# cvlab-yonsei/HVPR

Hardware: AMD Instinct MI355X
Metric: KITTI frames/sec/GPU (fwd, ~20k pts); VFE+scatter achieved HBM GB/s vs peak (higher is better)
Workload: dtype f32; 1 GPU; hvpr_car.yaml batch=1 forward-only, a1..a8 (on-GPU voxelize, pillar VFE, memory read-out + scatter, BEV backbone, head + decode, score top-k + rotated-BEV NMS); frames sharded over ranks, replicas only; global_batch=1, weights=deterministic synthetic (seed 0), BN stats randomised, cls bias -4.595

## Files before the change

### hvpr_amd/csrc/conv_wino.hip

```cpp
#include <type_traits>

#include "common.h"
#include "wino_walk.h"

namespace {

typedef float f32x16 __attribute__((ext_vector_type(16)));
constexpr int KC = 8;
constexpr int BN = 64;
constexpr int TW = 16, PW = TW + 2;
constexpr int ROWP = 20;
constexpr int W_V4 = 16 * 2 * BN;

__device__ __forceinline__ void lds_dma16(const void *sbase_uniform, unsigned voff_bytes, unsigned lds_dst_uniform) {
    unsigned keep;
    asm volatile("s_mov_b32 %0, m0\n\ts_mov_b32 m0, %3\n\ts_nop 0\n\tglobal_load_lds_dwordx4 %1, %2\n\ts_mov_b32 m0, %0"
                 : "=&s"(keep)
                 : "v"(voff_bytes), "s"(sbase_uniform), "s"(lds_dst_uniform)
                 : "memory");
}

__device__ __forceinline__ unsigned lds_addr_of(const void *p) {
    return (unsigned)(size_t)(const __attribute__((address_space(3))) void *)p;
}

struct WinoArgs {
    const float *in;
    const float *wpk;
    const float *bias;
    float *out;
    const float *gate;
    const float *resid;
    int N, H, W, Cin;
    int cout, cout_pad;
    int out_cstride, out_coff, resid_cstride;
    int relu;
    WinoWalk walk;
    int n_ct;
    float *stats;
};

__device__ __forceinline__ float4 f4_fma(float s, float4 a, float4 b) {
    return make_float4(fmaf(s, a.x, b.x), fmaf(s, a.y, b.y), fmaf(s, a.z, b.z), fmaf(s, a.w, b.w));
}
__device__ __forceinline__ float4 f4_add(float4 a, float4 b) { return make_float4(a.x + b.x, a.y + b.y, a.z + b.z, a.w + b.w); }
__device__ __forceinline__ float4 f4_sub(float4 a, float4 b) { return make_float4(a.x - b.x, a.y - b.y, a.z - b.z, a.w - b.w); }

template <int NG, bool STATS, int NB>
__global__ void __launch_bounds__(256 * NG) __attribute__((amdgpu_waves_per_eu(2, NB == 2 ? 2 : 3))) k_wino(WinoArgs a) {
    constexpr int NT = 256 * NG;
    constexpr int TH = 8 * NG, PH = TH + 2;
    constexpr int PPAD = (PH * ROWP + 63) / 64 * 64;
    constexpr int PATCH_V4 = 2 * PPAD;
    constexpr int BNT = 32 * NB, W_V4T = 16 * 2 * BNT;
    constexpr int NLD_P = (PATCH_V4 + NT - 1) / NT, NLD_W = W_V4T / NT;
    constexpr int PATCH_PAD = NLD_P * NT;
    constexpr bool PAIR = NG == 1 && NB == 2 && !STATS;
    constexpr int PH_S = PAIR ? 12 : PH, PW_S = PAIR ? 20 : PW;
    constexpr int BIAS_SLOT = PH_S * ROWP;
    static_assert(W_V4T % NT == 0 && (NB == 2 || NG == 1), "whole DMA pieces");
    extern __shared__ __attribute__((aligned(16))) float4 smem[];
    float4 *const s_w = smem;
    float4 *const s_patch = smem + 2 * W_V4T;

    const int tid = threadIdx.x, lane = tid & 63, wid = tid >> 6;
    const unsigned wave_s = __builtin_amdgcn_readfirstlane((unsigned)(threadIdx.x >> 6));
    const int grp = wid >> 2, wa = wid & 3;
    const int half = lane >> 5, l31 = lane & 31;
    const int by = l31 >> 3, bx = l31 & 7;

    int p_py[NLD_P], p_px[NLD_P], p_part[NLD_P];
    bool p_live[NLD_P], p_one[NLD_P];
#pragma unroll
    for (int i = 0; i < NLD_P; ++i) {
        const int v = tid + i * NT;
        const int plane = v / PPAD, slot = v % PPAD;
        const int y = slot / ROWP, rem = slot % ROWP;
        const int x = 2 * (rem % 10) + rem / 10;
        p_py[i] = y; p_px[i] = x; p_part[i] = plane * 4;
        p_live[i] = plane < 2 && y < PH_S && x < PW_S;
        p_one[i] = plane < 2 && y < PH && x < PW;
    }
    const int r0 = wa == 0 ? 0 : (wa == 2 ? 2 : 1), r1 = wa == 2 ? 1 : (wa == 3 ? 3 : 2);
    const float sgn = wa == 1 ? 1.f : -1.f;
    const int pbase = half * PPAD + (2 * (4 * grp + by)) * ROWP + bx;
    const int u_off = (wa * 4 * 2 + half) * BNT + l31;
    const unsigned lds_w0 = lds_addr_of(s_w) + wave_s * 1024u;
    const unsigned lds_patch0 = lds_addr_of(s_patch) + wave_s * 1024u;

    const int n_pt = a.walk.per_image * a.N;
    const int total_walk = ((n_pt + 7) / 8) * 8 * a.n_ct;
    const int n_chunks = a.Cin / KC;
    for (int it = blockIdx.x; it < total_walk; it += gridDim.x) {
    int ct;
    int pt = wino_walk_step(it, a.n_ct, ct);
    if (pt >= n_pt) continue;
    int tx, ty, n, mode = WINO_SINGLE;
    if constexpr (PAIR) {
        const WinoItem w = wino_walk_item(a.walk, pt);
        tx = w.tx; ty = w.ty; n = w.n; mode = w.mode;
    } else {
        tx = pt % a.walk.tiles_x; pt /= a.walk.tiles_x;
        ty = pt % a.walk.tiles_y;
        n = pt / a.walk.tiles_y;
    }
    const bool pr = PAIR && mode == WINO_PAIR_RIGHT, pb = PAIR && mode == WINO_PAIR_BOTTOM;
    const bool lane_b = pr ? bx >= 4 : (pb && by >= 2);
    const int p_off0 = pbase + r0 * ROWP + (lane_b ? (pr ? 1 : 2 * ROWP) : 0), p_off1 = p_off0 + (r1 - r0) * ROWP;
    const int oy0 = ty * TH, ox0 = tx * TW;
    const int iy0 = oy0 - 1, ix0 = ox0 - 1;
    const int co0 = ct * BNT;

    unsigned poff[NLD_P];
    bool pok[NLD_P];
#pragma unroll
    for (int i = 0; i < NLD_P; ++i) {
        int iy = iy0 + p_py[i], ix = ix0 + p_px[i];
        bool ok = PAIR ? p_one[i] : p_live[i];
        if (pr) { ok = p_live[i] && p_py[i] < PH; if (p_px[i] >= 10) { iy += TH; ix -= 10; } }
        if (pb) { ok = p_live[i] && p_px[i] < PW; if (p_py[i] >= 6) { iy -= 6; ix += TW; } }
        pok[i] = ok && iy >= 0 && iy < a.H && ix >= 0 && ix < a.W;
        poff[i] = pok[i] ? (unsigned)(((iy * a.W + ix) * a.Cin + p_part[i]) * (int)sizeof(float)) : 0u;
    }
    const char *in_n = (const char *)(a.in + (size_t)n * a.H * a.W * a.Cin);
    const char *w_ct = (const char *)(a.wpk + (size_t)(NB == 2 ? ct : ct >> 1) * n_chunks * (W_V4 * 4));
    const unsigned w_half = NB == 2 ? 0u : (unsigned)(ct & 1) * 32u * 16u;

    auto stage_piece = [&](int chunk, int buf, int i) {
        if (i < NLD_P) {
            const char *pbase_g = in_n + (size_t)chunk * (KC * sizeof(float));
            if (pok[i]) lds_dma16(pbase_g, poff[i], lds_patch0 + (unsigned)(buf * PATCH_PAD + i * NT) * 16u);
        } else {
            const int j = i - NLD_P;
            const char *wbase = w_ct + (size_t)chunk * (W_V4 * 16);
            lds_dma16(wbase, NB == 2 ? (unsigned)((tid + j * NT) * 16) : (unsigned)((((tid + j * NT) >> 5) * 64 + ((tid + j * NT) & 31)) * 16) + w_half,
                      lds_w0 + (unsigned)(buf * W_V4T + j * NT) * 16u);
        }
    };
    auto stage = [&](int chunk, int buf) {
#pragma unroll
        for (int i = 0; i < NLD_P + NLD_W; ++i) stage_piece(chunk, buf, i);
    };
    const bool border = pr || pb || iy0 < 0 || ix0 < 0 || iy0 + PH > a.H || ix0 + PW > a.W;
    if (border) {
#pragma unroll
        for (int b = 0; b < 2; ++b)
#pragma unroll
            for (int i = 0; i < NLD_P; ++i) s_patch[b * PATCH_PAD + tid + i * NT] = make_float4(0.f, 0.f, 0.f, 0.f);
        __syncthreads();
    }
    static_assert(BIAS_SLOT + BNT / 4 <= PPAD, "room for the bias row behind the patch");
    if (tid < BNT / 4) s_patch[BIAS_SLOT + tid] = *(const float4 *)(a.bias + co0 + tid * 4);
    f32x16 acc[4][NB];
#pragma unroll
    for (int b = 0; b < 4; ++b)
#pragma unroll
        for (int nb = 0; nb < NB; ++nb)
#pragma unroll
            for (int r = 0; r < 16; ++r) acc[b][nb][r] = 0.f;

    auto chunk_step = [&](int c, auto buf_tag) {
        constexpr int BUF = decltype(buf_tag)::value;
        asm volatile("s_waitcnt vmcnt(0)" ::: "memory");
        __builtin_amdgcn_s_barrier();
        const float4 *sp = s_patch + BUF * PATCH_PAD;
        const float4 *sw = s_w + BUF * W_V4T;
        float4 d0[4], d1[4], u[4][NB];
#pragma unroll
        for (int jx = 0; jx < 4; ++jx) {
            d0[jx] = sp[p_off0 + (jx & 1) * 10 + (jx >> 1)];
            d1[jx] = sp[p_off1 + (jx & 1) * 10 + (jx >> 1)];
        }
#pragma unroll
        for (int b = 0; b < 2; ++b)
#pragma unroll
            for (int nb = 0; nb < NB; ++nb) u[b][nb] = sw[u_off + b * 2 * BNT + nb * 32];
        __builtin_amdgcn_sched_barrier(0);
        float4 t[4], v[4];
#pragma unroll
        for (int jx = 0; jx < 4; ++jx) t[jx] = f4_fma(sgn, d1[jx], d0[jx]);
        v[0] = f4_sub(t[0], t[2]); v[1] = f4_add(t[1], t[2]); v[2] = f4_sub(t[2], t[1]); v[3] = f4_sub(t[1], t[3]);
#pragma unroll
        for (int b = 0; b < 4; ++b) {
            if (b + 2 < 4) {
#pragma unroll
                for (int nb = 0; nb < NB; ++nb) u[b + 2][nb] = sw[u_off + (b + 2) * 2 * BNT + nb * 32];
            }
            __builtin_amdgcn_sched_barrier(0);
#pragma unroll
            for (int nb = 0; nb < NB; ++nb) {
                acc[b][nb] = __builtin_amdgcn_mfma_f32_32x32x2f32(u[b][nb].x, v[b].x, acc[b][nb], 0, 0, 0);
                acc[b][nb] = __builtin_amdgcn_mfma_f32_32x32x2f32(u[b][nb].y, v[b].y, acc[b][nb], 0, 0, 0);
                acc[b][nb] = __builtin_amdgcn_mfma_f32_32x32x2f32(u[b][nb].z, v[b].z, acc[b][nb], 0, 0, 0);
                acc[b][nb] = __builtin_amdgcn_mfma_f32_32x32x2f32(u[b][nb].w, v[b].w, acc[b][nb], 0, 0, 0);
                constexpr int DEAL = 4 * NB > 5 ? 5 : 4 * NB - 1, NPF = (NLD_P + NLD_W + DEAL - 1) / DEAL;
                static_assert(DEAL * NPF >= NLD_P + NLD_W, "every piece goes out");
                if (c + 1 < n_chunks && b * NB + nb < DEAL) {
                    __builtin_amdgcn_sched_barrier(0);
#pragma unroll
                    for (int i = (b * NB + nb) * NPF; i < (b * NB + nb + 1) * NPF && i < NLD_P + NLD_W; ++i) stage_piece(c + 1, BUF ^ 1, i);
                    __builtin_amdgcn_sched_barrier(0);
                }
            }
            __builtin_amdgcn_sched_barrier(0);
        }
    };
    stage(0, 0);
    for (int c = 0; c + 1 < n_chunks; c += 2) {
        chunk_step(c, std::integral_constant<int, 0>{});
        chunk_step(c + 1, std::integral_constant<int, 1>{});
    }
    if (n_chunks & 1) chunk_step(n_chunks - 1, std::integral_constant<int, 0>{});

    const int p = wa >> 1, q = wa & 1;
    const int oy = oy0 + 2 * (4 * grp + by) + p + (lane_b ? (pr ? TH : -4) : 0), ox = ox0 + 2 * bx + q + (lane_b ? (pr ? -8 : TW) : 0);
    const bool live_px = oy < a.H && ox < a.W;
    const size_t pix = ((size_t)n * a.H + (live_px ? oy : 0)) * a.W + (live_px ? ox : 0);
    const float gate = a.gate && live_px ? a.gate[pix] : 0.f;
    const float *rrow = a.gate ? a.resid + pix * a.resid_cstride : nullptr;
    const float sg = p ? -1.f : 1.f;
    constexpr int NPASS = NG == 1 ? 1 : 2, NBP = NB / NPASS;
    float4 ykeep[2][4];
#pragma unroll
    for (int i = 0; i < 8; ++i) ykeep[i >> 2][i & 3] = make_float4(0.f, 0.f, 0.f, 0.f);
#pragma unroll
    for (int ps = 0; ps < NPASS; ++ps) {
        __syncthreads();
#pragma unroll
        for (int nl = 0; nl < NBP; ++nl) {
            const int nb = ps * NBP + nl;
#pragma unroll
            for (int g = 0; g < 4; ++g) {
                float4 m[4];
#pragma unroll
                for (int b = 0; b < 4; ++b) m[b] = make_float4(acc[b][nb][4 * g], acc[b][nb][4 * g + 1], acc[b][nb][4 * g + 2], acc[b][nb][4 * g + 3]);
                s_w[((((grp * 4 + wa) * 2 + 0) * NBP + nl) * 4 + g) * 64 + lane] = f4_add(f4_add(m[0], m[1]), m[2]);
                s_w[((((grp * 4 + wa) * 2 + 1) * NBP + nl) * 4 + g) * 64 + lane] = f4_sub(f4_sub(m[1], m[2]), m[3]);
            }
        }
        __syncthreads();
        if (live_px) {
#pragma unroll
            for (int nl = 0; nl < NBP; ++nl) {
                const int nb = ps * NBP + nl;
#pragma unroll
                for (int g = 0; g < 4; ++g) {
                    const int col = co0 + nb * 32 + 8 * g + 4 * half;
                    if (col >= a.cout) continue;
                    const float4 x0 = s_w[((((grp * 4 + p) * 2 + q) * NBP + nl) * 4 + g) * 64 + lane];
                    const float4 x1 = s_w[((((grp * 4 + p + 1) * 2 + q) * NBP + nl) * 4 + g) * 64 + lane];
                    const float4 x2 = s_w[((((grp * 4 + p + 2) * 2 + q) * NBP + nl) * 4 + g) * 64 + lane];
                    const float4 bias = s_patch[BIAS_SLOT + (col - co0) / 4];
                    float4 y = f4_add(f4_fma(sg, x2, f4_fma(sg, x1, x0)), bias);
                    if (a.relu) { y.x = fmaxf(y.x, 0.f); y.y = fmaxf(y.y, 0.f); y.z = fmaxf(y.z, 0.f); y.w = fmaxf(y.w, 0.f); }
                    if (a.gate) {
                        const float4 r = *(const float4 *)(rrow + col);
                        y.x = fmaf(gate, y.x, r.x); y.y = fmaf(gate, y.y, r.y); y.z = fmaf(gate, y.z, r.z); y.w = fmaf(gate, y.w, r.w);
                    }
                    *(float4 *)(a.out + pix * a.out_cstride + a.out_coff + col) = y;
                    if (STATS) ykeep[nl][g] = y;
                }
            }
        }
    }
    static_assert(!STATS || (NG == 1 && NB == 2), "the statistics pass is written for the 8 x 16 px x 64 channel tile");
    if (STATS) {
        __syncthreads();
#pragma unroll
        for (int nl = 0; nl < 2; ++nl)
#pragma unroll
            for (int g = 0; g < 4; ++g) s_w[((wid * 2 + nl) * 4 + g) * 64 + lane] = ykeep[nl][g];
        __syncthreads();
        {
            const int c = tid & 63, part = tid >> 6;
            const float *base = (const float *)(s_w + ((part * 2 + (c >> 5)) * 4 + ((c >> 3) & 3)) * 64 + ((c >> 2) & 1) * 32) + (c & 3);
            float sm = 0.f, sq = 0.f;
#pragma unroll 8
            for (int i = 0; i < 32; ++i) {
                const float v = base[((i + c) & 31) * 4];
                sm += v; sq = fmaf(v, v, sq);
            }
            float *s_part = (float *)(s_w + 2048);
            s_part[(part * 2 + 0) * 64 + c] = sm;
            s_part[(part * 2 + 1) * 64 + c] = sq;
        }
        __syncthreads();
        if (tid < 128) {
            const float *s_part = (const float *)(s_w + 2048);
            const int c = tid & 63, k = tid >> 6;
            const float v = (s_part[(0 * 2 + k) * 64 + c] + s_part[(1 * 2 + k) * 64 + c]) + (s_part[(2 * 2 + k) * 64 + c] + s_part[(3 * 2 + k) * 64 + c]);
            const int pt_lin = (n * a.walk.tiles_y + ty) * a.walk.tiles_x + tx;
            if (co0 + c < a.cout) a.stats[((size_t)pt_lin * 2 + k) * a.cout + co0 + c] = v;
        }
    }
    __syncthreads();
    }
}

__global__ void k_wino_pack(const float *__restrict__ w, const float *__restrict__ scale, int cout, int cin, int cout_pad, int adjoint,
                            float *__restrict__ out) {
    const long long id = blockIdx.x * (long long)blockDim.x + threadIdx.x;
    if (id >= (long long)cout_pad * cin) return;
    const int o = (int)(id / cin), i = (int)(id % cin);
    double g[3][3];
#pragma unroll
    for (int u = 0; u < 3; ++u)
#pragma unroll
        for (int v = 0; v < 3; ++v) {
            double x = 0.0;
            if (o < cout) x = adjoint ? (double)w[(((size_t)i * cout + o) * 3 + (2 - u)) * 3 + (2 - v)] : (double)w[(((size_t)o * cin + i) * 3 + u) * 3 + v];
            g[u][v] = (scale && o < cout) ? x * (double)scale[o] : x;
        }
    double gg[4][3];
#pragma unroll
    for (int v = 0; v < 3; ++v) {
        gg[0][v] = g[0][v];
        gg[1][v] = 0.5 * (g[0][v] + g[1][v] + g[2][v]);
        gg[2][v] = 0.5 * (g[0][v] - g[1][v] + g[2][v]);
        gg[3][v] = g[2][v];
    }
    const int ct = o / BN, co_l = o % BN, chunk = i / KC, hf = (i % KC) / 4, e = i % 4;
    float *dst = out + ((size_t)ct * (cin / KC) + chunk) * (W_V4 * 4);
#pragma unroll
    for (int r = 0; r < 4; ++r) {
        const double U[4] = {gg[r][0], 0.5 * (gg[r][0] + gg[r][1] + gg[r][2]), 0.5 * (gg[r][0] - gg[r][1] + gg[r][2]), gg[r][2]};
#pragma unroll
        for (int b = 0; b < 4; ++b) dst[(((size_t)(r * 4 + b) * 2 + hf) * BN + co_l) * 4 + e] = (float)U[b];
    }
}

template <int NG, bool STATS, int NB>
int launch(WinoArgs a, hipStream_t s) {
    constexpr int NT = 256 * NG, TH = 8 * NG, PH = TH + 2;
    constexpr int PPAD = (PH * ROWP + 63) / 64 * 64;
    constexpr int NLD_P = (2 * PPAD + NT - 1) / NT;
    constexpr int lds = (2 * (16 * 2 * 32 * NB) + 2 * NLD_P * NT) * 16;
    a.walk = wino_walk_make(a.H, a.W, TH, NG == 1 && NB == 2 && !STATS);
    a.n_ct = a.cout_pad / (32 * NB);
    static unsigned long long lds_set = 0ull;
    if (hvpr_ensure_dyn_lds((const void *)k_wino<NG, STATS, NB>, lds, &lds_set) != 0) return -1;
    const long long tiles = (long long)a.N * a.walk.per_image * a.n_ct;
    static int resident = 0;
    if (resident == 0) {
        int per_cu = 0, dev = 0, cus = 256;
        hipDeviceProp_t prop;
        if (hipGetDevice(&dev) == hipSuccess && hipGetDeviceProperties(&prop, dev) == hipSuccess) cus = prop.multiProcessorCount;
        if (hipOccupancyMaxActiveBlocksPerMultiprocessor(&per_cu, k_wino<NG, STATS, NB>, NT, lds) != hipSuccess || per_cu < 1) per_cu = 1;
        resident = per_cu * cus;
    }
    long long blocks = tiles < resident ? (tiles + 7) / 8 * 8 : resident;
    if (blocks > resident && resident >= 8) blocks = resident / 8 * 8;
    hipLaunchKernelGGL((k_wino<NG, STATS, NB>), dim3((unsigned)blocks), dim3(NT), lds, s, a);
    return 0;
}

}

extern "C" int hvpr_conv2d_wino_stats_rows(int N, int H, int W) {
    if (N < 1 || H < 1 || W < 1) return 0;
    return N * ((H + 7) / 8) * ((W + TW - 1) / TW);
}

extern "C" int hvpr_conv2d_wino_items(int N, int H, int W, int cout, int px_groups) {
    if (N < 1 || H < 1 || W < 1 || cout < 1 || (px_groups != 1 && px_groups != 2 && px_groups != 4)) return 0;
    const WinoWalk w = wino_walk_make(H, W, px_groups == 2 ? 16 : 8, px_groups == 1);
    const long long items = (long long)N * w.per_image * ((cout + BN - 1) / BN * BN / (px_groups == 4 ? 32 : 64));
    return items < (1ll << 31) ? (int)items : 0;
}

extern "C" size_t hvpr_conv2d_wino_packed_floats(int cin, int cout) {
    if (cin < 1 || cout < 1) return 0;
    return (size_t)((cout + BN - 1) / BN * BN) * (size_t)cin * 16;
}

extern "C" int hvpr_conv2d_wino_pack_f32(const float *weight, const float *scale, int cout, int cin, int adjoint, float *packed,
                                         hvpr_stream_t stream) {
    if (!weight || !packed || cout < 1 || cin < 1) return HVPR_ERR_INVALID_ARG;
    if (cin % KC != 0) return HVPR_ERR_UNSUPPORTED;
    const int cout_pad = (cout + BN - 1) / BN * BN;
    const long long n = (long long)cout_pad * cin;
    hipLaunchKernelGGL(k_wino_pack, dim3(hvpr_cdiv(n, 256)), dim3(256), 0, (hipStream_t)stream, weight, scale, cout, cin, cout_pad,
                       adjoint ? 1 : 0, packed);
    HVPR_CHECK_LAUNCH();
    return HVPR_OK;
}

extern "C" int hvpr_conv2d_wino_nhwc_f32(const float *in, int N, int H, int W, int Cin, const float *w_packed, const float *bias,
                                         int cout, int relu, const float *gate, const float *resid, int resid_cstride, float *out,
                                         int out_cstride, int out_coff, int px_groups, float *bn_partials, hvpr_stream_t stream) {
    if (!in || !w_packed || !bias || !out || N < 1 || H < 1 || W < 1 || Cin < 8 || cout < 1) return HVPR_ERR_INVALID_ARG;
    if ((gate == nullptr) != (resid == nullptr)) return HVPR_ERR_INVALID_ARG;
    if (Cin % KC != 0) return HVPR_ERR_UNSUPPORTED;
    if (cout % 4 != 0 || out_cstride % 4 != 0 || out_coff % 4 != 0 || (resid && resid_cstride % 4 != 0)) return HVPR_ERR_UNSUPPORTED;
    if ((long long)H * W * Cin * 4 >= (1ll << 31)) return HVPR_ERR_UNSUPPORTED;
    WinoArgs a;
    a.in = in; a.wpk = w_packed; a.bias = bias; a.out = out; a.gate = gate; a.resid = resid;
    a.N = N; a.H = H; a.W = W; a.Cin = Cin;
    a.cout = cout; a.cout_pad = (cout + BN - 1) / BN * BN;
    a.out_cstride = out_cstride; a.out_coff = out_coff; a.resid_cstride = resid_cstride;
    a.relu = relu;
    a.stats = bn_partials;
    if (bn_partials && (px_groups != 1 || relu || gate)) return HVPR_ERR_UNSUPPORTED;
    int rc;
    if (px_groups == 1) rc = bn_partials ? launch<1, true, 2>(a, (hipStream_t)stream) : launch<1, false, 2>(a, (hipStream_t)stream);
    else if (px_groups == 2) rc = launch<2, false, 2>(a, (hipStream_t)stream);
    else if (px_groups == 4) rc = launch<1, false, 1>(a, (hipStream_t)stream);
    else return HVPR_ERR_INVALID_ARG;
    if (rc != 0) return HVPR_ERR_LAUNCH;
    HVPR_CHECK_LAUNCH();
    return HVPR_OK;
}
```

### hvpr_amd/csrc/wino_walk.h

```cpp
#pragma once

#if defined(__HIPCC__) || defined(__CUDACC__)
#define HVPR_WALK_HD __host__ __device__ __forceinline__
#else
#define HVPR_WALK_HD inline
#endif

enum { WINO_SINGLE = 0, WINO_PAIR_RIGHT = 1, WINO_PAIR_BOTTOM = 2 };

struct WinoWalk {
    int tiles_x, tiles_y;
    int wi, hi;
    int n_plain, n_right;
    int per_image;
};

struct WinoItem {
    int n;
    int mode;
    int ty, tx;
};

HVPR_WALK_HD WinoWalk wino_walk_make(int H, int W, int tile_h, int pairing) {
    WinoWalk w;
    w.tiles_x = (W + 15) / 16;
    w.tiles_y = (H + tile_h - 1) / tile_h;
    const int live_bcols = (W - 16 * (w.tiles_x - 1) + 1) / 2;
    const int live_brows = (H - tile_h * (w.tiles_y - 1) + 1) / 2;
    const int rp = pairing && tile_h == 8 && live_bcols <= 4, bp = pairing && tile_h == 8 && live_brows <= 2;
    w.wi = rp ? w.tiles_x - 1 : w.tiles_x;
    w.hi = bp ? w.tiles_y - 1 : w.tiles_y;
    w.n_plain = w.wi * w.hi;
    w.n_right = rp ? (w.tiles_y + 1) / 2 : 0;
    w.per_image = w.n_plain + w.n_right + (bp ? (w.wi + 1) / 2 : 0);
    return w;
}

HVPR_WALK_HD int wino_walk_step(int it, int n_ct, int &ct) {
    const int xcd = it & 7, j = it >> 3;
    ct = j % n_ct;
    return (j / n_ct) * 8 + xcd;
}

HVPR_WALK_HD WinoItem wino_walk_item(const WinoWalk &w, int pt) {
    WinoItem it;
    it.n = pt / w.per_image;
    int q = pt - it.n * w.per_image;
    if (q < w.n_plain) {
        it.ty = q / w.wi; it.tx = q - it.ty * w.wi; it.mode = WINO_SINGLE;
    } else if ((q -= w.n_plain) < w.n_right) {
        it.ty = 2 * q; it.tx = w.tiles_x - 1;
        it.mode = it.ty + 1 < w.tiles_y ? WINO_PAIR_RIGHT : WINO_SINGLE;
    } else {
        q -= w.n_right;
        it.ty = w.tiles_y - 1; it.tx = 2 * q;
        it.mode = it.tx + 1 < w.wi ? WINO_PAIR_BOTTOM : WINO_SINGLE;
    }
    return it;
}
```

Baseline: 458.6 frames/s.

## Overlap Winograd prologue DMA with border zero-fill and restructure epilogue

Issues the first chunk's patch and weight DMA before the border zero-fill. Zero-fills only the patch slots that DMA will not write, which removes the barrier between fill and staging. Loads the bias row into a register early. The epilogue now computes both output-transform halves in registers, prefetches gate and residual values before the barrier, and cuts the per-pass barriers down. It also adds opt-in s_memtime instrumentation behind a compile flag, and moves the patch-slot helpers into a header.

```diff
diff --git a/hvpr_amd/csrc/conv_wino.hip b/hvpr_amd/csrc/conv_wino.hip
--- a/hvpr_amd/csrc/conv_wino.hip
+++ b/hvpr_amd/csrc/conv_wino.hip
@@ -8,8 +8,8 @@
 typedef float f32x16 __attribute__((ext_vector_type(16)));
 constexpr int KC = 8;
 constexpr int BN = 64;
-constexpr int TW = 16, PW = TW + 2;
-constexpr int ROWP = 20;
+constexpr int TW = WINO_TW, PW = TW + 2;
+constexpr int ROWP = WINO_ROWP;
 constexpr int W_V4 = 16 * 2 * BN;
 
 __device__ __forceinline__ void lds_dma16(const void *sbase_uniform, unsigned voff_bytes, unsigned lds_dst_uniform) {
@@ -40,6 +40,14 @@
     float *stats;
 };
 
+#ifdef HVPR_EXP_TIMING
+constexpr int WD_BLOCKS = 1024, WD_ITEMS = 4;
+__device__ unsigned long long g_wino_dbg[WD_BLOCKS * WD_ITEMS * 8];
+#define WD_STAMP(k) asm volatile("s_memtime %0\n s_waitcnt lgkmcnt(0)" : "=s"(wd_t[k]) :: "memory")
+#else
+#define WD_STAMP(k)
+#endif
+
 __device__ __forceinline__ float4 f4_fma(float s, float4 a, float4 b) {
     return make_float4(fmaf(s, a.x, b.x), fmaf(s, a.y, b.y), fmaf(s, a.z, b.z), fmaf(s, a.w, b.w));
 }
@@ -56,7 +64,7 @@
     constexpr int NLD_P = (PATCH_V4 + NT - 1) / NT, NLD_W = W_V4T / NT;
     constexpr int PATCH_PAD = NLD_P * NT;
     constexpr bool PAIR = NG == 1 && NB == 2 && !STATS;
-    constexpr int PH_S = PAIR ? 12 : PH, PW_S = PAIR ? 20 : PW;
+    constexpr int PH_S = PAIR ? 12 : PH;
     constexpr int BIAS_SLOT = PH_S * ROWP;
     static_assert(W_V4T % NT == 0 && (NB == 2 || NG == 1), "whole DMA pieces");
     extern __shared__ __attribute__((aligned(16))) float4 smem[];
@@ -70,16 +78,14 @@
     const int by = l31 >> 3, bx = l31 & 7;
 
     int p_py[NLD_P], p_px[NLD_P], p_part[NLD_P];
-    bool p_live[NLD_P], p_one[NLD_P];
+    bool p_plane[NLD_P];
 #pragma unroll
     for (int i = 0; i < NLD_P; ++i) {
         const int v = tid + i * NT;
-        const int plane = v / PPAD, slot = v % PPAD;
-        const int y = slot / ROWP, rem = slot % ROWP;
-        const int x = 2 * (rem % 10) + rem / 10;
-        p_py[i] = y; p_px[i] = x; p_part[i] = plane * 4;
-        p_live[i] = plane < 2 && y < PH_S && x < PW_S;
-        p_one[i] = plane < 2 && y < PH && x < PW;
+        const int plane = v / PPAD;
+        wino_patch_slot(v % PPAD, p_py[i], p_px[i]);
+        p_part[i] = plane * 4;
+        p_plane[i] = plane < 2;
     }
     const int r0 = wa == 0 ? 0 : (wa == 2 ? 2 : 1), r1 = wa == 2 ? 1 : (wa == 3 ? 3 : 2);
     const float sgn = wa == 1 ? 1.f : -1.f;
@@ -91,10 +97,27 @@
     const int n_pt = a.walk.per_image * a.N;
     const int total_walk = ((n_pt + 7) / 8) * 8 * a.n_ct;
     const int n_chunks = a.Cin / KC;
+#ifdef HVPR_EXP_TIMING
+    int wd_item = 0;
+#endif
     for (int it = blockIdx.x; it < total_walk; it += gridDim.x) {
     int ct;
     int pt = wino_walk_step(it, a.n_ct, ct);
     if (pt >= n_pt) continue;
+#ifdef HVPR_EXP_TIMING
+    unsigned long long wd_t[7];
+#endif
+    WD_STAMP(0);
+    const int co0 = ct * BNT;
+    const char *w_ct = (const char *)(a.wpk + (size_t)(NB == 2 ? ct : ct >> 1) * n_chunks * (W_V4 * 4));
+    const unsigned w_half = NB == 2 ? 0u : (unsigned)(ct & 1) * 32u * 16u;
+    auto stage_w = [&](int chunk, int buf, int j) {
+        const char *wbase = w_ct + (size_t)chunk * (W_V4 * 16);
+        lds_dma16(wbase, NB == 2 ? (unsigned)((tid + j * NT) * 16) : (unsigned)((((tid + j * NT) >> 5) * 64 + ((tid + j * NT) & 31)) * 16) + w_half,
+                  lds_w0 + (unsigned)(buf * W_V4T + j * NT) * 16u);
+    };
+    float4 bias_row = make_float4(0.f, 0.f, 0.f, 0.f);
+    if (tid < BNT / 4) bias_row = *(const float4 *)(a.bias + co0 + tid * 4);
     int tx, ty, n, mode = WINO_SINGLE;
     if constexpr (PAIR) {
         const WinoItem w = wino_walk_item(a.walk, pt);
@@ -109,48 +132,39 @@
     const int p_off0 = pbase + r0 * ROWP + (lane_b ? (pr ? 1 : 2 * ROWP) : 0), p_off1 = p_off0 + (r1 - r0) * ROWP;
     const int oy0 = ty * TH, ox0 = tx * TW;
     const int iy0 = oy0 - 1, ix0 = ox0 - 1;
-    const int co0 = ct * BNT;
 
     unsigned poff[NLD_P];
-    bool pok[NLD_P];
+    bool pok[NLD_P], pzero[NLD_P];
 #pragma unroll
     for (int i = 0; i < NLD_P; ++i) {
-        int iy = iy0 + p_py[i], ix = ix0 + p_px[i];
-        bool ok = PAIR ? p_one[i] : p_live[i];
-        if (pr) { ok = p_live[i] && p_py[i] < PH; if (p_px[i] >= 10) { iy += TH; ix -= 10; } }
-        if (pb) { ok = p_live[i] && p_px[i] < PW; if (p_py[i] >= 6) { iy -= 6; ix += TW; } }
-        pok[i] = ok && iy >= 0 && iy < a.H && ix >= 0 && ix < a.W;
+        int iy, ix;
+        pok[i] = p_plane[i] && wino_patch_dma_writes(mode, TH, p_py[i], p_px[i], oy0, ox0, a.H, a.W, iy, ix);
+        pzero[i] = p_plane[i] && wino_patch_fills(mode, TH, p_py[i], p_px[i], oy0, ox0, a.H, a.W);
         poff[i] = pok[i] ? (unsigned)(((iy * a.W + ix) * a.Cin + p_part[i]) * (int)sizeof(float)) : 0u;
     }
     const char *in_n = (const char *)(a.in + (size_t)n * a.H * a.W * a.Cin);
-    const char *w_ct = (const char *)(a.wpk + (size_t)(NB == 2 ? ct : ct >> 1) * n_chunks * (W_V4 * 4));
-    const unsigned w_half = NB == 2 ? 0u : (unsigned)(ct & 1) * 32u * 16u;
 
     auto stage_piece = [&](int chunk, int buf, int i) {
         if (i < NLD_P) {
             const char *pbase_g = in_n + (size_t)chunk * (KC * sizeof(float));
             if (pok[i]) lds_dma16(pbase_g, poff[i], lds_patch0 + (unsigned)(buf * PATCH_PAD + i * NT) * 16u);
         } else {
-            const int j = i - NLD_P;
-            const char *wbase = w_ct + (size_t)chunk * (W_V4 * 16);
-            lds_dma16(wbase, NB == 2 ? (unsigned)((tid + j * NT) * 16) : (unsigned)((((tid + j * NT) >> 5) * 64 + ((tid + j * NT) & 31)) * 16) + w_half,
-                      lds_w0 + (unsigned)(buf * W_V4T + j * NT) * 16u);
+            stage_w(chunk, buf, i - NLD_P);
         }
     };
-    auto stage = [&](int chunk, int buf) {
-#pragma unroll
-        for (int i = 0; i < NLD_P + NLD_W; ++i) stage_piece(chunk, buf, i);
-    };
+#pragma unroll
+    for (int i = 0; i < NLD_P + NLD_W; ++i) stage_piece(0, 0, i);
+    WD_STAMP(1);
+    __builtin_amdgcn_sched_barrier(0);
     const bool border = pr || pb || iy0 < 0 || ix0 < 0 || iy0 + PH > a.H || ix0 + PW > a.W;
     if (border) {
 #pragma unroll
-        for (int b = 0; b < 2; ++b)
-#pragma unroll
-            for (int i = 0; i < NLD_P; ++i) s_patch[b * PATCH_PAD + tid + i * NT] = make_float4(0.f, 0.f, 0.f, 0.f);
-        __syncthreads();
-    }
-    static_assert(BIAS_SLOT + BNT / 4 <= PPAD, "room for the bias row behind the patch");
-    if (tid < BNT / 4) s_patch[BIAS_SLOT + tid] = *(const float4 *)(a.bias + co0 + tid * 4);
+        for (int i = 0; i < NLD_P; ++i)
+            if (pzero[i]) {
+                s_patch[tid + i * NT] = make_float4(0.f, 0.f, 0.f, 0.f);
+                s_patch[PATCH_PAD + tid + i * NT] = make_float4(0.f, 0.f, 0.f, 0.f);
+            }
+    }
     f32x16 acc[4][NB];
 #pragma unroll
     for (int b = 0; b < 4; ++b)
@@ -163,6 +177,9 @@
         constexpr int BUF = decltype(buf_tag)::value;
         asm volatile("s_waitcnt vmcnt(0)" ::: "memory");
         __builtin_amdgcn_s_barrier();
+#ifdef HVPR_EXP_TIMING
+        if (c == 0) WD_STAMP(2);
+#endif
         const float4 *sp = s_patch + BUF * PATCH_PAD;
         const float4 *sw = s_w + BUF * W_V4T;
         float4 d0[4], d1[4], u[4][NB];
@@ -205,64 +222,105 @@
             __builtin_amdgcn_sched_barrier(0);
         }
     };
-    stage(0, 0);
+    static_assert(BIAS_SLOT + BNT / 4 <= PPAD, "room for the bias row behind the patch");
+    if (tid < BNT / 4) s_patch[BIAS_SLOT + tid] = bias_row;
+    asm volatile("s_waitcnt lgkmcnt(0)" ::: "memory");
     for (int c = 0; c + 1 < n_chunks; c += 2) {
         chunk_step(c, std::integral_constant<int, 0>{});
         chunk_step(c + 1, std::integral_constant<int, 1>{});
     }
     if (n_chunks & 1) chunk_step(n_chunks - 1, std::integral_constant<int, 0>{});
 
+    WD_STAMP(3);
     const int p = wa >> 1, q = wa & 1;
     const int oy = oy0 + 2 * (4 * grp + by) + p + (lane_b ? (pr ? TH : -4) : 0), ox = ox0 + 2 * bx + q + (lane_b ? (pr ? -8 : TW) : 0);
     const bool live_px = oy < a.H && ox < a.W;
     const size_t pix = ((size_t)n * a.H + (live_px ? oy : 0)) * a.W + (live_px ? ox : 0);
-    const float gate = a.gate && live_px ? a.gate[pix] : 0.f;
-    const float *rrow = a.gate ? a.resid + pix * a.resid_cstride : nullptr;
+    constexpr int NPASS = NG == 1 ? 1 : 2, NBP = NB / NPASS;
+    float4 *const xg = s_w + grp * (4 * 2 * NBP * 4 * 64) + lane;
+    auto xoff = [](int arow, int qq, int nl, int g) { return (((arow * 2 + qq) * NBP + nl) * 4 + g) * 64; };
+    const int col0 = co0 + 4 * half;
+    const float4 *const sbias = s_patch + BIAS_SLOT + half;
+    float *const orow = a.out + pix * a.out_cstride + a.out_coff + col0;
+    float gate = 0.f;
+    float4 rres[NB][4];
+    float4 ykeep[2][4];
     const float sg = p ? -1.f : 1.f;
-    constexpr int NPASS = NG == 1 ? 1 : 2, NBP = NB / NPASS;
-    float4 ykeep[2][4];
-#pragma unroll
-    for (int i = 0; i < 8; ++i) ykeep[i >> 2][i & 3] = make_float4(0.f, 0.f, 0.f, 0.f);
-#pragma unroll
-    for (int ps = 0; ps < NPASS; ++ps) {
-        __syncthreads();
+    const float4 *const xr = xg + xoff(p, q, 0, 0);
+    auto finish = [&](int ps) {
 #pragma unroll
         for (int nl = 0; nl < NBP; ++nl) {
             const int nb = ps * NBP + nl;
 #pragma unroll
             for (int g = 0; g < 4; ++g) {
+                const int cg = nb * 32 + 8 * g;
+                if (col0 >= a.cout - cg) continue;
+                float4 x[3];
+#pragma unroll
+                for (int k = 0; k < 3; ++k) x[k] = xr[xoff(k, 0, nl, g)];
+                const float4 bias = sbias[cg / 4];
+                float4 y = f4_add(f4_fma(sg, x[2], f4_fma(sg, x[1], x[0])), bias);
+                if (a.relu) { y.x = fmaxf(y.x, 0.f); y.y = fmaxf(y.y, 0.f); y.z = fmaxf(y.z, 0.f); y.w = fmaxf(y.w, 0.f); }
+                if (a.gate) {
+                    asm volatile("");
+                    const float4 rs = rres[nb][g];
+                    y.x = fmaf(gate, y.x, rs.x); y.y = fmaf(gate, y.y, rs.y); y.z = fmaf(gate, y.z, rs.z); y.w = fmaf(gate, y.w, rs.w);
+                }
+                *(float4 *)(orow + cg) = y;
+                if (STATS) ykeep[nl][g] = y;
+            }
+        }
+    };
+#pragma unroll
+    for (int ps = 0; ps < NPASS; ++ps) {
+        float4 r[NBP][4][2];
+#pragma unroll
+        for (int nl = 0; nl < NBP; ++nl) {
+            const int nb = ps * NBP + nl;
+#pragma unroll
+            for (int g = 0; g < 4; ++g) {
                 float4 m[4];
 #pragma unroll
                 for (int b = 0; b < 4; ++b) m[b] = make_float4(acc[b][nb][4 * g], acc[b][nb][4 * g + 1], acc[b][nb][4 * g + 2], acc[b][nb][4 * g + 3]);
-                s_w[((((grp * 4 + wa) * 2 + 0) * NBP + nl) * 4 + g) * 64 + lane] = f4_add(f4_add(m[0], m[1]), m[2]);
-                s_w[((((grp * 4 + wa) * 2 + 1) * NBP + nl) * 4 + g) * 64 + lane] = f4_sub(f4_sub(m[1], m[2]), m[3]);
+                r[nl][g][0] = f4_add(f4_add(m[0], m[1]), m[2]);
+                r[nl][g][1] = f4_sub(f4_sub(m[1], m[2]), m[3]);
+            }
+        }
+        if (ps == 0) {
+#pragma unroll
+            for (int i = 0; i < NBP * 4 * 2; ++i) {
+                float4 &v = r[i >> 3][(i >> 1) & 3][i & 1];
+                asm volatile("" : "+v"(v.x), "+v"(v.y), "+v"(v.z), "+v"(v.w));
+            }
+#pragma unroll
+            for (int i = 0; i < NB * 4; ++i) {
+                float4 &v = rres[i >> 2][i & 3];
+                asm volatile("" : "=v"(v.x), "=v"(v.y), "=v"(v.z), "=v"(v.w));
+            }
+            if (a.gate && live_px) {
+                gate = a.gate[pix];
+                const float *rrow = a.resid + pix * a.resid_cstride + col0;
+#pragma unroll
+                for (int nb = 0; nb < NB; ++nb)
+#pragma unroll
+                    for (int g = 0; g < 4; ++g) {
+                        const int cg = nb * 32 + 8 * g;
+                        if (col0 < a.cout - cg) rres[nb][g] = *(const float4 *)(rrow + cg);
+                    }
             }
         }
         __syncthreads();
-        if (live_px) {
-#pragma unroll
-            for (int nl = 0; nl < NBP; ++nl) {
-                const int nb = ps * NBP + nl;
-#pragma unroll
-                for (int g = 0; g < 4; ++g) {
-                    const int col = co0 + nb * 32 + 8 * g + 4 * half;
-                    if (col >= a.cout) continue;
-                    const float4 x0 = s_w[((((grp * 4 + p) * 2 + q) * NBP + nl) * 4 + g) * 64 + lane];
-                    const float4 x1 = s_w[((((grp * 4 + p + 1) * 2 + q) * NBP + nl) * 4 + g) * 64 + lane];
-                    const float4 x2 = s_w[((((grp * 4 + p + 2) * 2 + q) * NBP + nl) * 4 + g) * 64 + lane];
-                    const float4 bias = s_patch[BIAS_SLOT + (col - co0) / 4];
-                    float4 y = f4_add(f4_fma(sg, x2, f4_fma(sg, x1, x0)), bias);
-                    if (a.relu) { y.x = fmaxf(y.x, 0.f); y.y = fmaxf(y.y, 0.f); y.z = fmaxf(y.z, 0.f); y.w = fmaxf(y.w, 0.f); }
-                    if (a.gate) {
-                        const float4 r = *(const float4 *)(rrow + col);
-                        y.x = fmaf(gate, y.x, r.x); y.y = fmaf(gate, y.y, r.y); y.z = fmaf(gate, y.z, r.z); y.w = fmaf(gate, y.w, r.w);
-                    }
-                    *(float4 *)(a.out + pix * a.out_cstride + a.out_coff + col) = y;
-                    if (STATS) ykeep[nl][g] = y;
-                }
-            }
-        }
-    }
+#pragma unroll
+        for (int i = 0; i < NBP * 4 * 2; ++i) xg[xoff(0, i & 1, i >> 3, (i >> 1) & 3) + wa * (2 * NBP * 4 * 64)] = r[i >> 3][(i >> 1) & 3][i & 1];
+        if (ps == NPASS - 1) WD_STAMP(4);
+        __syncthreads();
+        if (STATS) {
+#pragma unroll
+            for (int i = 0; i < 8; ++i) ykeep[i >> 2][i & 3] = make_float4(0.f, 0.f, 0.f, 0.f);
+        }
+        if (live_px) finish(ps);
+    }
+    WD_STAMP(5);
     static_assert(!STATS || (NG == 1 && NB == 2), "the statistics pass is written for the 8 x 16 px x 64 channel tile");
     if (STATS) {
         __syncthreads();
@@ -294,6 +352,16 @@
         }
     }
     __syncthreads();
+#ifdef HVPR_EXP_TIMING
+    WD_STAMP(6);
+    if (tid == 0 && blockIdx.x < WD_BLOCKS && wd_item < WD_ITEMS) {
+        unsigned long long *d = g_wino_dbg + ((size_t)blockIdx.x * WD_ITEMS + wd_item) * 8;
+#pragma unroll
+        for (int k = 0; k < 7; ++k) d[k] = wd_t[k];
+        d[7] = 1ull | (border ? 2ull : 0ull) | ((unsigned long long)mode << 2) | (a.gate ? 16ull : 0ull);
+    }
+    ++wd_item;
+#endif
     }
 }
 
@@ -355,6 +423,16 @@
 }
 
 }
+
+#ifdef HVPR_EXP_TIMING
+extern "C" int hvpr_exp_wino_dbg(unsigned long long *host_out, int n_words) {
+    void *dev = nullptr;
+    if (hipDeviceSynchronize() != hipSuccess || hipGetSymbolAddress(&dev, HIP_SYMBOL(g_wino_dbg)) != hipSuccess) return -1;
+    if (n_words < 0 || (size_t)n_words > sizeof(g_wino_dbg) / 8) return -1;
+    if (hipMemcpy(host_out, dev, sizeof(unsigned long long) * n_words, hipMemcpyDeviceToHost) != hipSuccess) return -1;
+    return hipMemset(dev, 0, sizeof(g_wino_dbg)) == hipSuccess ? 0 : -1;
+}
+#endif
 
 extern "C" int hvpr_conv2d_wino_stats_rows(int N, int H, int W) {
     if (N < 1 || H < 1 || W < 1) return 0;
diff --git a/hvpr_amd/csrc/wino_walk.h b/hvpr_amd/csrc/wino_walk.h
--- a/hvpr_amd/csrc/wino_walk.h
+++ b/hvpr_amd/csrc/wino_walk.h
@@ -58,3 +58,36 @@
     }
     return it;
 }
+
+enum { WINO_ROWP = 20, WINO_TW = 16 };
+
+HVPR_WALK_HD void wino_patch_slot(int slot, int &y, int &x) {
+    const int rem = slot % WINO_ROWP;
+    y = slot / WINO_ROWP;
+    x = 2 * (rem % 10) + rem / 10;
+}
+
+HVPR_WALK_HD bool wino_patch_pixel(int mode, int tile_h, int y, int x, int &dy, int &dx) {
+    dy = y; dx = x;
+    if (mode == WINO_PAIR_RIGHT) {
+        if (x >= 10) { dy = y + tile_h; dx = x - 10; }
+        return y < tile_h + 2 && x < 20;
+    }
+    if (mode == WINO_PAIR_BOTTOM) {
+        if (y >= 6) { dy = y - 6; dx = x + WINO_TW; }
+        return y < 12 && x < WINO_TW + 2;
+    }
+    return y < tile_h + 2 && x < WINO_TW + 2;
+}
+
+HVPR_WALK_HD bool wino_patch_dma_writes(int mode, int tile_h, int y, int x, int oy0, int ox0, int H, int W, int &iy, int &ix) {
+    int dy, dx;
+    const bool staged = wino_patch_pixel(mode, tile_h, y, x, dy, dx);
+    iy = oy0 - 1 + dy; ix = ox0 - 1 + dx;
+    return staged && iy >= 0 && iy < H && ix >= 0 && ix < W;
+}
+
+HVPR_WALK_HD bool wino_patch_fills(int mode, int tile_h, int y, int x, int oy0, int ox0, int H, int W) {
+    int dy, dx, iy, ix;
+    return wino_patch_pixel(mode, tile_h, y, x, dy, dx) && !wino_patch_dma_writes(mode, tile_h, y, x, oy0, ox0, H, W, iy, ix);
+}
```

New measurement: 454.1 frames/s. About the same (-1.0%).
